# gue-ni/raytracer.glsl

Measured on AMD Instinct MI355X. Metric: Mpaths/s at 1920x1080, 8 bounces, 10k tris, higher is better.
Workload: dtype f32; 1 GPU; C2: 1920x1080, 8 bounces, 10000 triangles + 5 spheres, cube map 256^2, 1 spp/frame progressive, dof=1; parallelism=1 GPU(s), 8-row strips interleaved, gather to rank 0 every frame, frame_batch=1, kernel=4, wf_rays=4, wf_mode=1, wf_chunk=256, wf_early=0, wf_packed=0, mf_sets=4, mf_group_quads=32, mf_chunk_quads=32

## Files before the change

raytracer.glsl_amd/csrc/rt_mfma.hpp:

```cpp
#pragma once
#include "rt_wavefront.hpp"

#pragma clang fp contract(off)

namespace rt {

typedef __bf16 bf16x8 __attribute__((ext_vector_type(8)));
typedef float f32x16 __attribute__((ext_vector_type(16)));

constexpr int kMfTileTris = 10;
constexpr int kMfQuadTiles = 4;
constexpr int kMfQuadTris = kMfTileTris * kMfQuadTiles;
constexpr uint32_t kMfMaxChunkQuads = 32;
constexpr uint32_t kMfMaxGroupQuads = 64;

struct alignas(16) MfGroup {
    float cx, cy, cz;
    float E;
    float Ml;
    float Pw;
    float P;
    float pad1;
};

// ... 107 lines not shown

__device__ __forceinline__ float mf_margin(const MfGroup &G, float ncv, float no, const MfRay &r)
{
    float local = __builtin_fmaf(0.00396728515625f * G.E, ncv, 6.103515625e-05f * (G.Ml * r.wd));
    float cancel = 9.5367431640625e-07f * (__builtin_fmaf(G.E, no, G.P) * r.wd);
    float world = 9.5367431640625e-07f * __builtin_fmaf(G.E, r.wod, G.Pw * r.wd);
    return (local + cancel) + (world + 1e-30f);
}

struct alignas(16) MfCull {
    float cx, cy, cz, R;
    float ax, ay, az, Rc;
    float t1x, t1y, t1z, X;
    float t2x, t2y, t2z, Y;
    float Nmin, shape, hmin, lmax;
    float Pw, inv_len;
    float iB, iB2;
    float iB_lo, iB2_lo, pad0, pad1;
};
static_assert(sizeof(MfCull) == 112, "seven uint4 per tile");

__device__ __forceinline__ float wave_sum(float x) { for (int off = 32; off > 0; off >>= 1) x += __shfl_xor(x, off); return x; }

__global__ void __launch_bounds__(64) prepare_cull_kernel(const float4 *__restrict__ vertices, const uint32_t *__restrict__ visit_tri,
                                                          const uint32_t *__restrict__ order, uint32_t n_visits, uint32_t n_tiles, MfCull *__restrict__ out)
{
    const uint32_t q = blockIdx.x, lane = threadIdx.x;
    if (q >= n_tiles) return;
    const uint32_t pos = q * kMfTileTris + lane;
    const bool have = lane < (uint32_t)kMfTileTris && pos < n_visits;
    const float inf = __builtin_inff();
    f3 w[3] = {mk(0.0f, 0.0f, 0.0f), mk(0.0f, 0.0f, 0.0f), mk(0.0f, 0.0f, 0.0f)};
    if (have) { const uint32_t tri = visit_tri[order[pos]]; for (int k = 0; k < 3; ++k) { const float4 p = vertices[3 * (size_t)tri + k]; w[k] = mk(p.x, p.y, p.z); } }
    f3 lo = mk(inf, inf, inf), hi = mk(-inf, -inf, -inf);
    bool bad = false;
    if (have) for (int k = 0; k < 3; ++k) {
        lo = mk(fminf(lo.x, w[k].x), fminf(lo.y, w[k].y), fminf(lo.z, w[k].z));
        hi = mk(fmaxf(hi.x, w[k].x), fmaxf(hi.y, w[k].y), fmaxf(hi.z, w[k].z));
        bad |= !(fabsf(w[k].x) < 1e18f) || !(fabsf(w[k].y) < 1e18f) || !(fabsf(w[k].z) < 1e18f);
    }
    lo = mk(wave_min(lo.x), wave_min(lo.y), wave_min(lo.z));
    hi = mk(wave_max(hi.x), wave_max(hi.y), wave_max(hi.z));
    const f3 c = mk(0.5f * lo.x + 0.5f * hi.x, 0.5f * lo.y + 0.5f * hi.y, 0.5f * lo.z + 0.5f * hi.z);
    float R = 0.0f, Rc = 0.0f, E = 0.0f, Pw = 0.0f, Nmin = inf, shape = inf, hmin = inf;
    f3 nh = mk(0.0f, 0.0f, 0.0f);
    if (have) {
        const f3 e0 = w[1] - w[0], e1 = w[2] - w[1], e2 = w[0] - w[2];
        const f3 N = cross3(e0, mk(-e2.x, -e2.y, -e2.z));
        const float nn = __builtin_sqrtf(dot3(N, N));
        const float l0 = __builtin_sqrtf(dot3(e0, e0)), l1 = __builtin_sqrtf(dot3(e1, e1)), l2 = __builtin_sqrtf(dot3(e2, e2));
        for (int k = 0; k < 3; ++k) { const f3 r = w[k] - c; R = fmaxf(R, __builtin_sqrtf(dot3(r, r))); }
        { const f3 g = mk((w[0].x + w[1].x + w[2].x) * (1.0f / 3.0f), (w[0].y + w[1].y + w[2].y) * (1.0f / 3.0f), (w[0].z + w[1].z + w[2].z) * (1.0f / 3.0f)) - c;
          Rc = __builtin_sqrtf(dot3(g, g)); }
        E = fmaxf(l0, fmaxf(l1, l2));
        const float a0 = __builtin_sqrtf(dot3(w[0], w[0])), a1 = __builtin_sqrtf(dot3(w[1], w[1])), a2 = __builtin_sqrtf(dot3(w[2], w[2]));
        Pw = fmaxf(a0 * a1, fmaxf(a1 * a2, a2 * a0));
        Nmin = nn;
        nh = (nn > 0.0f) ? mk(N.x / nn, N.y / nn, N.z / nn) : mk(0.0f, 0.0f, 0.0f);
        const float c0 = -dot3(e0, e2) / (l0 * l2), c1 = -dot3(e1, e0) / (l1 * l0), c2 = -dot3(e2, e1) / (l2 * l1);
        const float cmax = fminf(1.0f, fmaxf(c0, fmaxf(c1, c2)));
        const float s = __builtin_sqrtf(fmaxf(0.0f, 0.5f * (1.0f - cmax)));
        const float lmin = fminf(l0, fminf(l1, l2));
        shape = (nn > 0.0f) ? 0.999f * s * lmin / nn : 0.0f;
        if (!(shape == shape)) shape = 0.0f;
        hmin = (E > 0.0f) ? 0.999f * nn / E : 0.0f;
        if (!(hmin == hmin)) hmin = 0.0f;
    }
    R = wave_max(R); Rc = wave_max(Rc); E = wave_max(E); Pw = wave_max(Pw); Nmin = wave_min(Nmin); shape = wave_min(shape); hmin = wave_min(hmin);
    bad = __any(bad) || __any(have && !(nh.x == nh.x && nh.y == nh.y && nh.z == nh.z));
    f3 a = mk(wave_sum(have ? nh.x : 0.0f), wave_sum(have ? nh.y : 0.0f), wave_sum(have ? nh.z : 0.0f));
    const float al = __builtin_sqrtf(dot3(a, a));
    a = (al > 0.0f) ? mk(a.x / al, a.y / al, a.z / al) : mk(0.0f, 0.0f, 1.0f);
    const float ca = have ? dot3(nh, a) : 1.0f;
    bad |= !(al > 0.0f) || __any(have && !(ca > 0.1f));
    const f3 ref = (fabsf(a.x) < 0.7f) ? mk(1.0f, 0.0f, 0.0f) : mk(0.0f, 1.0f, 0.0f);
    f3 b1 = cross3(a, ref);
    { const float bl = __builtin_sqrtf(dot3(b1, b1)); b1 = mk(b1.x / bl, b1.y / bl, b1.z / bl); }
    const f3 b2 = cross3(a, b1);
    const float ica = 1.0f / fmaxf(ca, 0.1f);
    const float gu = have ? dot3(nh, b1) * ica : 0.0f, gv = have ? dot3(nh, b2) * ica : 0.0f;
    const float suu = wave_sum(gu * gu), suv = wave_sum(gu * gv), svv = wave_sum(gv * gv);
    const float phi = 0.5f * atan2f(2.0f * suv, suu - svv);
    const float cp = cosf(phi), sp = sinf(phi);
    f3 t1 = mk(cp * b1.x + sp * b2.x, cp * b1.y + sp * b2.y, cp * b1.z + sp * b2.z);
    { const float tl = __builtin_sqrtf(dot3(t1, t1)); t1 = mk(t1.x / tl, t1.y / tl, t1.z / tl); }
    f3 t2 = cross3(a, t1);
    { const float tl = __builtin_sqrtf(dot3(t2, t2)); t2 = mk(t2.x / tl, t2.y / tl, t2.z / tl); }
    const float X = wave_max(have ? fabsf(dot3(nh, t1) * ica) : 0.0f), Y = wave_max(have ? fabsf(dot3(nh, t2) * ica) : 0.0f);
    if (lane != 0) return;
    MfCull rec;
    rec.cx = c.x; rec.cy = c.y; rec.cz = c.z; rec.R = R * 1.0001f + 1e-30f;
    rec.ax = a.x; rec.ay = a.y; rec.az = a.z; rec.Rc = Rc * 1.0001f + 1e-30f;
    rec.t1x = t1.x; rec.t1y = t1.y; rec.t1z = t1.z; rec.X = X * 1.001f + 1e-5f;
    rec.t2x = t2.x; rec.t2y = t2.y; rec.t2z = t2.z; rec.Y = Y * 1.001f + 1e-5f;
    bad |= !(rec.X < 16.0f) || !(rec.Y < 16.0f);
    rec.Nmin = bad ? 0.0f : Nmin * 0.999f; rec.shape = bad ? 0.0f : shape; rec.hmin = bad ? 0.0f : hmin; rec.lmax = E * 1.001f;
    rec.Pw = Pw * 1.001f;
    rec.inv_len = 0.9999f / __builtin_sqrtf(1.0f + rec.X * rec.X + rec.Y * rec.Y);
    rec.iB = 1.0001f / (1.0f + rec.X * rec.X); rec.iB2 = 1.0001f / (1.0f + rec.Y * rec.Y);
    rec.iB_lo = 0.9999f / (1.0f + rec.X * rec.X); rec.iB2_lo = 0.9999f / (1.0f + rec.Y * rec.Y);
    rec.pad0 = rec.pad1 = 0.0f;
    out[q] = rec;
}

struct MfPacket { f3 O, D; float ro, sigma, On; };

__device__ __forceinline__ float mf_max_dot(const MfCull &c, float wa, float w1, float w2, float wn)
{
    const bool inside = (wa > 0.0f) && (w1 <= c.X * wa) && (w2 <= c.Y * wa);
    const float num = __builtin_fmaf(c.Y, w2, __builtin_fmaf(c.X, w1, wa));
    const float corner = num * c.inv_len * (num > 0.0f ? 1.0003f : 1.0f);
// ... 49 lines not shown
```

raytracer.glsl_amd/csrc/rt_scan.hpp:

```cpp
#pragma once
#include <type_traits>
#include "rt_mfma.hpp"

#pragma clang fp contract(off)

namespace rt {

typedef uint32_t u32x4 __attribute__((ext_vector_type(4)));
typedef float f32x6 __attribute__((ext_vector_type(6)));

template <bool kMax> __device__ __forceinline__ float half_reduce(float x)
{
    auto op = [](float a, float b) { return kMax ? __builtin_fmaxf(a, b) : __builtin_fminf(a, b); };
    auto dpp = [](float v, auto ctrl) { return __builtin_bit_cast(float, __builtin_amdgcn_update_dpp(0, __builtin_bit_cast(int, v), decltype(ctrl)::value, 0xf, 0xf, false)); };
    x = op(x, dpp(x, std::integral_constant<int, 0xB1>{}));
    x = op(x, dpp(x, std::integral_constant<int, 0x4E>{}));
    x = op(x, dpp(x, std::integral_constant<int, 0x141>{}));
    x = op(x, dpp(x, std::integral_constant<int, 0x140>{}));
    const float r0 = __builtin_bit_cast(float, __builtin_amdgcn_readlane(__builtin_bit_cast(int, x), 0));
    const float r1 = __builtin_bit_cast(float, __builtin_amdgcn_readlane(__builtin_bit_cast(int, x), 16));
    return op(r0, r1);
}
__device__ __forceinline__ float half_max(float x) { return half_reduce<true>(x); }
__device__ __forceinline__ float half_min(float x) { return half_reduce<false>(x); }
template <bool kMax> __device__ __forceinline__ float full_reduce(float x)
{
    auto op = [](float a, float b) { return kMax ? __builtin_fmaxf(a, b) : __builtin_fminf(a, b); };
    auto dpp = [](float v, auto ctrl) { return __builtin_bit_cast(float, __builtin_amdgcn_update_dpp(0, __builtin_bit_cast(int, v), decltype(ctrl)::value, 0xf, 0xf, false)); };
    x = op(x, dpp(x, std::integral_constant<int, 0xB1>{}));
    x = op(x, dpp(x, std::integral_constant<int, 0x4E>{}));
    x = op(x, dpp(x, std::integral_constant<int, 0x141>{}));
    x = op(x, dpp(x, std::integral_constant<int, 0x140>{}));
    auto rl = [&](int l) { return __builtin_bit_cast(float, __builtin_amdgcn_readlane(__builtin_bit_cast(int, x), l)); };
    return op(op(rl(0), rl(16)), op(rl(32), rl(48)));
}

__global__ void __launch_bounds__(256) packet_cull_kernel(WaveBuffers wb, const MfCull *__restrict__ cull, uint32_t n_tiles, uint32_t bounce, float ro_add, float sigma_add)
{
    const uint32_t n_rays = wb.counts[bounce];
    const RayQueue qin = (bounce & 1u) ? wb.q[1] : wb.q[0];
    const uint32_t lane = threadIdx.x & 63u, n_gran = (n_rays + 127u) / 128u;
    const float inf = __builtin_inff();
    for (uint32_t g = blockIdx.x * 4u + (threadIdx.x >> 6); g < n_gran; g += gridDim.x * 4u) {
        f3 o[2], dh[2]; bool valid[2]; bool usable = true;
        f3 olo = mk(inf, inf, inf), ohi = mk(-inf, -inf, -inf), dlo = olo, dhi = ohi;
#pragma unroll
        for (int k = 0; k < 2; ++k) {
            const uint32_t slot = g * 128u + (uint32_t)k * 64u + lane;
            valid[k] = slot < n_rays;
            o[k] = mk(0.0f, 0.0f, 0.0f); dh[k] = o[k];
            if (valid[k]) {
                const float4 a = qin.a[slot], b = qin.b[slot];
                o[k] = mk(a.x, a.y, a.z);
                const f3 d = mk(a.w, b.x, b.y);
                const float dd = dot3(d, d), il = __builtin_amdgcn_rsqf(dd), dl = dd * il;
                dh[k] = mk(d.x * il, d.y * il, d.z * il);
                usable &= (dl > 0.0f) && (dl < inf) && (fabsf(o[k].x) < 1e18f) && (fabsf(o[k].y) < 1e18f) && (fabsf(o[k].z) < 1e18f);
                olo = mk(fminf(olo.x, o[k].x), fminf(olo.y, o[k].y), fminf(olo.z, o[k].z)); ohi = mk(fmaxf(ohi.x, o[k].x), fmaxf(ohi.y, o[k].y), fmaxf(ohi.z, o[k].z));
                dlo = mk(fminf(dlo.x, dh[k].x), fminf(dlo.y, dh[k].y), fminf(dlo.z, dh[k].z)); dhi = mk(fmaxf(dhi.x, dh[k].x), fmaxf(dhi.y, dh[k].y), fmaxf(dhi.z, dh[k].z));
            }
        }
        olo = mk(full_reduce<false>(olo.x), full_reduce<false>(olo.y), full_reduce<false>(olo.z)); ohi = mk(full_reduce<true>(ohi.x), full_reduce<true>(ohi.y), full_reduce<true>(ohi.z));
        dlo = mk(full_reduce<false>(dlo.x), full_reduce<false>(dlo.y), full_reduce<false>(dlo.z)); dhi = mk(full_reduce<true>(dhi.x), full_reduce<true>(dhi.y), full_reduce<true>(dhi.z));
        MfPacket pk;
        pk.O = mk(0.5f * olo.x + 0.5f * ohi.x, 0.5f * olo.y + 0.5f * ohi.y, 0.5f * olo.z + 0.5f * ohi.z);
        f3 D = mk(0.5f * dlo.x + 0.5f * dhi.x, 0.5f * dlo.y + 0.5f * dhi.y, 0.5f * dlo.z + 0.5f * dhi.z);
        const float DD = dot3(D, D), iDl = __builtin_amdgcn_rsqf(DD), Dl = DD * iDl;
        pk.D = mk(D.x * iDl, D.y * iDl, D.z * iDl);
        float ro = 0.0f, sigma = 0.0f;
#pragma unroll
        for (int k = 0; k < 2; ++k)
            if (valid[k]) {
                const f3 eo = o[k] - pk.O, ed = dh[k] - pk.D;
                ro = fmaxf(ro, __builtin_amdgcn_sqrtf(dot3(eo, eo))); sigma = fmaxf(sigma, __builtin_amdgcn_sqrtf(dot3(ed, ed)));
            }
        pk.ro = full_reduce<true>(ro) * 1.0001f + 1e-30f + ro_add; pk.sigma = full_reduce<true>(sigma) * 1.0001f + 2e-6f + sigma_add;
        usable = !__any(!usable) && (Dl > 0.25f);
        pk.On = __builtin_amdgcn_sqrtf(dot3(pk.O, pk.O)) * 1.0001f + pk.ro;
        uint32_t *const row = wb.keep + (size_t)g * wb.keep_words;
        MfCull c_next = {};
        bool have_next = usable && lane < n_tiles;
        if (have_next) c_next = cull[lane];
        for (uint32_t t0 = 0; t0 < n_tiles; t0 += 64u) {
            const MfCull c = c_next;
            const bool have_this = have_next;
            have_next = usable && t0 + 64u + lane < n_tiles;
            if (have_next) c_next = cull[t0 + 64u + lane];
            bool skip = false, open = false;
            f3 W = mk(0.0f, 0.0f, 0.0f); float L = 0.0f, nz = 0.0f, Wn = 0.0f;
            if (have_this && c.Nmin > 0.0f) {
                const f3 gq = pk.O - mk(c.cx, c.cy, c.cz);
                L = __builtin_amdgcn_sqrtf(dot3(gq, gq)) * 1.0001f;
                nz = 9.5367431640625e-07f * __builtin_fmaf(c.lmax, pk.On, c.Pw) * 1.01f;
                W = cross3(pk.D, gq);
                Wn = __builtin_amdgcn_sqrtf(dot3(W, W));
                skip = mf_certified_ka(c, pk, gq, L, nz, Wn);
                open = !skip;
            }
            if (__any(open)) { if (open) skip = mf_certified_b(c, pk, W, L, nz, Wn); }
            const unsigned long long have = (n_tiles - t0 >= 64u) ? ~0ull : ((1ull << (n_tiles - t0)) - 1ull);
            const unsigned long long keep = ~(unsigned long long)__builtin_amdgcn_ballot_w64(skip) & have;
            if (lane == 0u) {
                store_through(row + (t0 >> 5), (uint32_t)keep);
                if ((t0 >> 5) + 1u < wb.keep_words) store_through(row + ((t0 >> 5) + 1u), (uint32_t)(keep >> 32));
            }
        }
    }
}

__device__ __forceinline__ void exact_and_merge_at(const MfView &mf, const RayQueue &qin, unsigned long long *best, uint32_t slot, uint32_t pos)
{
    const float4 a = qin.a[slot], b = qin.b[slot];
    const uint32_t v = mf.order[pos];
    TriRay tr; tr.o = mk(a.x, a.y, a.z); tr.d = mk(a.w, b.x, b.y); tr.cv = cross3(tr.d, tr.o); tr.ncv = tr.nd = 0.0f;
    const float t = tri_exact(mf.edges_s[pos], mf.planes_s[pos], tr);
    if (kEps < t && t < kInf) atomicMin(&best[slot], ((unsigned long long)__float_as_uint(t) << 32) | v);
}

constexpr int kSoloSets = 4;
struct SoloCfg {
    static constexpr uint32_t kStepMax = 2u * 64u;
    static constexpr uint32_t kDrain = 192u;
// ... 668 lines not shown
```

raytracer.glsl_amd/csrc/rtgl_amd.hip:

```cpp
#include <hip/hip_runtime.h>
#include <algorithm>
#include <cmath>
#include <cstdio>
#include <cstring>
#include <string>
#include <vector>
#include <map>
#include <mutex>
#include <thread>
#include <condition_variable>
#include <memory>

#include "../../include/rtgl_amd.h"
#include "rt_device.hpp"
#include "rt_wavefront.hpp"
#include "rt_mfma.hpp"
#include "rt_scan.hpp"

#pragma clang fp contract(off)

using namespace rt;


__global__ void __launch_bounds__(256) prepare_triangles_kernel(const float4 *__restrict__ vertices,
// ... 125 lines not shown
    hipEvent_t ev0 = nullptr, ev1 = nullptr;
    bool timed = false;
    std::vector<hipEvent_t> kev;
    uint32_t kev_used = 0;
    std::vector<uint32_t> kev_frame_start;
    std::string error;

    std::vector<uint8_t> h_meshes, h_nodes, h_vertices;
    uint32_t n_meshes = 0, n_nodes = 0, n_vec4 = 0;

    SphereRec *d_spheres = nullptr; uint32_t n_spheres = 0;
    MaterialRec *d_materials = nullptr; uint32_t n_materials = 0;
    float4 *d_vertices = nullptr;
    uint32_t *d_sphere_visits = nullptr; uint32_t n_sphere_visits = 0;
    TriEdges *d_edges = nullptr; TriPlane *d_planes = nullptr; uint32_t n_tri_visits = 0;
    TriEdges *d_edges_s = nullptr; TriPlane *d_planes_s = nullptr;
    uint8_t *d_env = nullptr; int env_w = 0, env_h = 0, env_c = 0, env_faces = 0;
    float4 *d_image_own = nullptr, *d_image = nullptr;
    uint4 *d_rng = nullptr;
    Counters *d_counters = nullptr;
    uchar4 *d_u8 = nullptr;

    float2 *d_group_bounds = nullptr;
    MfGroup *d_mf_groups = nullptr; MfCull *d_mf_cull = nullptr; uint4 *d_mf_A = nullptr; uint32_t *d_mf_order = nullptr; uint32_t n_mf_groups = 0, mf_group_quads = 32; uint32_t *d_dbg_log = nullptr;
    void *d_wave = nullptr; size_t wave_capacity = 0; bool wave_multi = false;
    uint32_t *d_counts = nullptr; uint32_t counts_capacity = 0;
    uint32_t *h_counts = nullptr;
    hipEvent_t counts_ev = nullptr; bool counts_pending = false, counts_valid = false;
    bool timing_this_frame = false; uint32_t timing_frame_counter = 0;
    int kernel_in_use = -1;
    int n_cus = 256;
    uint2 *d_items = nullptr; size_t items_capacity = 0;
    uint32_t *d_sched = nullptr; size_t sched_capacity = 0;
    uint32_t *d_keep = nullptr; size_t keep_capacity = 0;
    uint32_t *d_keep0 = nullptr; size_t keep0_capacity = 0; bool keep0_valid = false; FrameParams keep0_params{}; uint32_t keep0_n0 = 0, keep0_words = 0; uint64_t keep0_scene = 0;
    uint64_t scene_version = 0;
    void *d_plan = nullptr; size_t plan_capacity = 0;
    void *d_stage = nullptr; size_t stage_capacity = 0;
    uint32_t *d_sort_hist = nullptr; uint32_t sort_bits_alloc = 0;
    int sort_set = 0; uint32_t sort_set_bits = 0; bool sort_sets_clean = false;
    float mesh_lo[3] = {0.0f, 0.0f, 0.0f}, mesh_hi[3] = {0.0f, 0.0f, 0.0f}, mesh_ext = 0.0f;
    uint2 *d_cand = nullptr; uint32_t cand_regions = 0, cand_region_pairs = 0, cand_region_target = 0; bool cand_fixed = false;
    bool solo_attr_set = false;
    bool group_explicit = false;
    bool kernel_explicit = false;
    uint32_t counts_n0 = 0, counts_len = 0;
    std::vector<uint32_t> est_counts;
// ... 168 lines not shown
            double cyc = 0, ticks = 0;
            for (int b = 0; b < 64 && h[16 * b + 8]; ++b) {
                const unsigned long long *d = h + 16 * b;
                fprintf(stderr, "rtgl clock bounce %2d: %llu waves, %.0f shader cycles per wave over %.0f ticks of 10 ns: %.3f GHz\n", b, d[8], (double)d[0] / d[8], (double)d[14] / d[8], d[14] ? (double)d[0] / (double)d[14] * 0.1 : 0.0);
                cyc += (double)d[0]; ticks += (double)d[14];
            }
            if (ticks > 0) fprintf(stderr, "rtgl clock: in-kernel shader clock of scan_solo_kernel, wave-time weighted over all launches: %.3f GHz\n", cyc / ticks * 0.1);
        }
#endif
        std::vector<unsigned long long> pc(16 * 64 * 2 * 16);
        if (hipMemcpy(pc.data(), reinterpret_cast<unsigned long long *>(ctx->d_dbg_log) + 2048, pc.size() * 8, hipMemcpyDeviceToHost) == hipSuccess)
            for (int b = 0; b < 8; ++b) {
                double tot = 0, cnt = 0; int nch = 0;
                for (int c = 0; c < 64; ++c) { const unsigned long long *e = pc.data() + ((size_t)16 * b * 64 + c) * 2; if (e[1]) { tot += (double)e[0]; cnt += (double)e[1]; nch = c + 1; } }
                if (cnt == 0) continue;
                fprintf(stderr, "rtgl stamps bounce %2d: mean wave time per chunk / bounce mean:", b);
                for (int c = 0; c < nch; ++c) { const unsigned long long *e = pc.data() + ((size_t)16 * b * 64 + c) * 2; fprintf(stderr, " %.2f", e[1] ? ((double)e[0] / (double)e[1]) / (tot / cnt) : 0.0); }
                fprintf(stderr, "\n");
            }
    }
#endif
    void *ptrs[] = { ctx->d_spheres, ctx->d_materials, ctx->d_vertices, ctx->d_sphere_visits, ctx->d_edges, ctx->d_planes,
                     ctx->d_env, ctx->d_image_own, ctx->d_rng, ctx->d_counters, ctx->d_u8, ctx->d_group_bounds, ctx->d_wave, ctx->d_counts, ctx->d_mf_groups, ctx->d_mf_A, ctx->d_mf_order,
                     ctx->d_dbg_log, ctx->d_cand, ctx->d_keep0, ctx->d_plan, ctx->d_stage, ctx->d_sort_hist, ctx->d_mf_cull, ctx->d_keep, ctx->d_items, ctx->d_sched, ctx->d_edges_s, ctx->d_planes_s, ctx->d_batch_rad };
    for (void *p : ptrs) if (p) (void)hipFree(p);
    for (hipEvent_t e : ctx->kev) (void)hipEventDestroy(e);
    if (ctx->h_counts) (void)hipHostFree(ctx->h_counts);
    if (ctx->counts_ev) (void)hipEventDestroy(ctx->counts_ev);
    if (ctx->ev0) (void)hipEventDestroy(ctx->ev0);
    if (ctx->ev1) (void)hipEventDestroy(ctx->ev1);
    if (ctx->own_stream) release_device_stream(ctx->device, ctx->own_stream, ctx->own_stream_shared);
    delete ctx;
}

extern "C" const char *rtgl_last_error(const rtgl_context *ctx) { return ctx ? ctx->error.c_str() : g_create_error.c_str(); }

static int flush_pending(rtgl_context *ctx);
#define ENTER_NOFLUSH(ctx) do { if (!(ctx)) return RTGL_ERR_INVALID; HIPCHK(ctx, hipSetDevice((ctx)->device)); } while (0)
#define ENTER(ctx) do { ENTER_NOFLUSH(ctx); if (!(ctx)->pending.empty()) { const int rcf_ = flush_pending(ctx); if (rcf_) return rcf_; } } while (0)
#define FANOUT(ctx, call) do { if (!(ctx)->parts.empty()) { (ctx)->gathered = false; \
    for (rtgl_context *part : (ctx)->parts) { const int rc_ = (call); if (rc_) return fail(ctx, rc_, std::string("device ") + std::to_string(part->device) + ": " + part->error); } \
    return RTGL_OK; } } while (0)

extern "C" int rtgl_create_multi(rtgl_context **out, int width, int height, const int *devices, int n_devices, int strip_rows)
{
    if (!out) return fail(nullptr, RTGL_ERR_INVALID, "out is NULL");
    *out = nullptr;
// ... 237 lines not shown
    while (!todo.empty()) {
        const size_t lo = todo.back().first, hi = todo.back().second, m = hi - lo;
        todo.pop_back();
        if (m <= (size_t)kMfTileTris) continue;
        const size_t unit = m > group_tris ? group_tris : (m > (size_t)kMfQuadTris ? (size_t)kMfQuadTris : (size_t)kMfTileTris);
        const size_t nl = ((m / 2 + unit - 1) / unit) * unit;
        const int dims = m > group_tris ? 3 : 6;
        float bl[6], bh[6];
        for (int a = 0; a < dims; ++a) { bl[a] = 3.0e38f; bh[a] = -3.0e38f; }
        for (size_t i = lo; i < hi; ++i)
            for (int a = 0; a < dims; ++a) { const float c = pts[6 * (size_t)order[i] + a]; bl[a] = std::min(bl[a], c); bh[a] = std::max(bh[a], c); }
        int ax = 0;
        for (int a = 1; a < dims; ++a) if (bh[a] - bl[a] > bh[ax] - bl[ax]) ax = a;
        std::nth_element(order.begin() + lo, order.begin() + lo + nl, order.begin() + hi, [&](uint32_t p, uint32_t q) {
            const float cp = pts[6 * (size_t)p + ax], cq = pts[6 * (size_t)q + ax];
            return cp < cq || (cp == cq && p < q);
        });
        todo.emplace_back(lo, lo + nl);
        todo.emplace_back(lo + nl, hi);
    }
    return order;
}

static int rebuild_triangles(rtgl_context *ctx)
{
    std::vector<uint32_t> visit_tri;
    uint32_t n_tris = ctx->n_vec4 / 3;
    for (uint32_t m = 0; m < ctx->n_meshes; ++m) {
        uint32_t start, size;
        memcpy(&start, ctx->h_meshes.data() + (size_t)m * 16, 4);
        memcpy(&size, ctx->h_meshes.data() + (size_t)m * 16 + 4, 4);
        uint64_t end = std::min<uint64_t>((uint64_t)start + size, n_tris);
        for (uint64_t t = start; t < end; ++t) visit_tri.push_back((uint32_t)t);
    }
    if (ctx->d_edges) { HIPCHK(ctx, hipFree(ctx->d_edges)); ctx->d_edges = nullptr; }
    if (ctx->d_planes) { HIPCHK(ctx, hipFree(ctx->d_planes)); ctx->d_planes = nullptr; }
    ctx->n_tri_visits = (uint32_t)visit_tri.size();
    ctx->scene_version++;
    {
        float lo[3] = {3.0e38f, 3.0e38f, 3.0e38f}, hi[3] = {-3.0e38f, -3.0e38f, -3.0e38f};
        const float *vx = reinterpret_cast<const float *>(ctx->h_vertices.data());
        for (uint32_t t : visit_tri)
            for (int k = 0; k < 3; ++k)
                for (int a = 0; a < 3; ++a) { const float c = vx[(size_t)t * 12 + 4 * k + a]; if (c == c && c > -1.0e30f && c < 1.0e30f) { lo[a] = std::min(lo[a], c); hi[a] = std::max(hi[a], c); } }
        ctx->mesh_ext = 0.0f;
        for (int a = 0; a < 3; ++a) { ctx->mesh_lo[a] = lo[a] <= hi[a] ? lo[a] : 0.0f; ctx->mesh_hi[a] = lo[a] <= hi[a] ? hi[a] : 0.0f; if (lo[a] <= hi[a]) ctx->mesh_ext = std::max(ctx->mesh_ext, hi[a] - lo[a]); }
    }
    if (ctx->n_tri_visits) {
        uint32_t *d_visit = nullptr;
        HIPCHK(ctx, hipMalloc((void **)&d_visit, visit_tri.size() * 4));
        HIPCHK(ctx, hipMemcpyAsync(d_visit, visit_tri.data(), visit_tri.size() * 4, hipMemcpyHostToDevice, ctx->stream));
        HIPCHK(ctx, hipMalloc((void **)&ctx->d_edges, (size_t)ctx->n_tri_visits * sizeof(TriEdges)));
        HIPCHK(ctx, hipMalloc((void **)&ctx->d_planes, (size_t)ctx->n_tri_visits * sizeof(TriPlane)));
        dim3 grid((ctx->n_tri_visits + 255) / 256);
        hipLaunchKernelGGL(prepare_triangles_kernel, grid, dim3(256), 0, ctx->stream, ctx->d_vertices, d_visit, ctx->n_tri_visits, ctx->d_edges, ctx->d_planes);
        HIPCHK(ctx, hipGetLastError());
        if (ctx->d_group_bounds) { HIPCHK(ctx, hipFree(ctx->d_group_bounds)); ctx->d_group_bounds = nullptr; }
        uint32_t n_groups = (ctx->n_tri_visits + kBoundGroup - 1) / kBoundGroup;
        HIPCHK(ctx, hipMalloc((void **)&ctx->d_group_bounds, (size_t)n_groups * sizeof(float2)));
        hipLaunchKernelGGL(group_bounds_kernel, dim3(n_groups), dim3(64), 0, ctx->stream, ctx->d_edges, ctx->n_tri_visits, ctx->d_group_bounds);
        HIPCHK(ctx, hipGetLastError());
        if (ctx->d_mf_groups) { HIPCHK(ctx, hipFree(ctx->d_mf_groups)); ctx->d_mf_groups = nullptr; }
        if (ctx->d_mf_A) { HIPCHK(ctx, hipFree(ctx->d_mf_A)); ctx->d_mf_A = nullptr; }
        if (ctx->d_mf_order) { HIPCHK(ctx, hipFree(ctx->d_mf_order)); ctx->d_mf_order = nullptr; }
        if (ctx->d_mf_cull) { HIPCHK(ctx, hipFree(ctx->d_mf_cull)); ctx->d_mf_cull = nullptr; }
        if (ctx->d_edges_s) { HIPCHK(ctx, hipFree(ctx->d_edges_s)); ctx->d_edges_s = nullptr; }
        if (ctx->d_planes_s) { HIPCHK(ctx, hipFree(ctx->d_planes_s)); ctx->d_planes_s = nullptr; }
        ctx->mf_group_quads = ctx->group_explicit ? (uint32_t)ctx->opt_mf_group_quads : 32u;
        const uint32_t group_tris = ctx->mf_group_quads * kMfQuadTris;
        ctx->n_mf_groups = (ctx->n_tri_visits + group_tris - 1) / group_tris;
        const std::vector<uint32_t> order = kd_order(ctx, visit_tri, group_tris);
        HIPCHK(ctx, hipMalloc((void **)&ctx->d_mf_order, order.size() * 4));
        HIPCHK(ctx, hipMemcpyAsync(ctx->d_mf_order, order.data(), order.size() * 4, hipMemcpyHostToDevice, ctx->stream));
        HIPCHK(ctx, hipMalloc((void **)&ctx->d_edges_s, (size_t)ctx->n_tri_visits * sizeof(TriEdges)));
        HIPCHK(ctx, hipMalloc((void **)&ctx->d_planes_s, (size_t)ctx->n_tri_visits * sizeof(TriPlane)));
        hipLaunchKernelGGL(gather_storage_order_kernel, dim3((ctx->n_tri_visits + 255) / 256), dim3(256), 0, ctx->stream, ctx->d_edges, ctx->d_planes, ctx->d_mf_order,
                           ctx->n_tri_visits, ctx->d_edges_s, ctx->d_planes_s);
        HIPCHK(ctx, hipMalloc((void **)&ctx->d_mf_groups, (size_t)ctx->n_mf_groups * sizeof(MfGroup)));
        const size_t a_bytes = ((size_t)ctx->n_mf_groups * ctx->mf_group_quads + 1) * kMfQuadTiles * 64 * sizeof(uint4);
        if (a_bytes > 0xFFFF0000ull) return fail(ctx, RTGL_ERR_INVALID, "mesh too large for the 32-bit tile offsets of the matrix-core scan");
        HIPCHK(ctx, hipMalloc((void **)&ctx->d_mf_A, a_bytes));
        HIPCHK(ctx, hipMemsetAsync(ctx->d_mf_A, 0, a_bytes, ctx->stream));
        hipLaunchKernelGGL(prepare_mfma_kernel, dim3(ctx->n_mf_groups), dim3(64), 0, ctx->stream, ctx->d_vertices, d_visit,
                           ctx->d_mf_order, ctx->n_tri_visits, ctx->n_mf_groups, ctx->mf_group_quads, ctx->d_mf_groups, ctx->d_mf_A, getenv("RTGL_AMD_ROW_GAMMA") ? (float)atof(getenv("RTGL_AMD_ROW_GAMMA")) : 1.220703125e-4f);
        HIPCHK(ctx, hipGetLastError());
        const uint32_t n_tiles_all = ctx->n_mf_groups * ctx->mf_group_quads * (uint32_t)kMfQuadTiles, n_tiles_alloc = n_tiles_all + 128u;
        HIPCHK(ctx, hipMalloc((void **)&ctx->d_mf_cull, (size_t)n_tiles_alloc * sizeof(MfCull)));
        HIPCHK(ctx, hipMemsetAsync(ctx->d_mf_cull, 0, (size_t)n_tiles_alloc * sizeof(MfCull), ctx->stream));
        hipLaunchKernelGGL(prepare_cull_kernel, dim3(n_tiles_all), dim3(64), 0, ctx->stream, ctx->d_vertices, d_visit,
                           ctx->d_mf_order, ctx->n_tri_visits, n_tiles_all, ctx->d_mf_cull);
        HIPCHK(ctx, hipGetLastError());
        HIPCHK(ctx, hipStreamSynchronize(ctx->stream));
        HIPCHK(ctx, hipFree(d_visit));
    } else ctx->n_mf_groups = 0;
    ctx->tris_dirty = false;
    return RTGL_OK;
}

static void kev_mark(rtgl_context *ctx)
{
    if (!ctx->timing_this_frame) return;
    if (ctx->kev_used == ctx->kev.size()) { hipEvent_t e; if (hipEventCreate(&e) != hipSuccess) return; ctx->kev.push_back(e); }
    (void)hipEventRecord(ctx->kev[ctx->kev_used++], ctx->stream);
}

static uint32_t solo_chunks(const rtgl_context *ctx);
static uint32_t solo_regions(const rtgl_context *ctx) { return std::max<uint32_t>((uint32_t)ctx->n_cus, solo_chunks(ctx)) * 8u; }

static size_t counts_bytes(uint32_t capacity) { return (size_t)(capacity + 1u) * sizeof(uint32_t); }

static void set_bin_cells(rtgl_context *ctx)
{
    WaveBuffers &wb = ctx->wb;
    const uint32_t T = wb.sort_T;
// ... 228 lines not shown
                               reinterpret_cast<const void *>(&scan_solo_kernel<false, 2, 3>), reinterpret_cast<const void *>(&scan_solo_kernel<true, 2, 3>)}) {
            hipFuncAttributes fattr;
            HIPCHK(ctx, hipFuncGetAttributes(&fattr, fn));
            HIPCHK(ctx, hipFuncSetAttribute(fn, hipFuncAttributeMaxDynamicSharedMemorySize, (int)(160 * 1024 - fattr.sharedSizeBytes)));
        }
        ctx->solo_attr_set = true;
    }

    if (cull) {
        float ro_add = 0.0f, sigma_add = 0.0f;
        bool have_bits = false;
        if (bounce == 0 && cam && camera_keep_widening(*cam, &ro_add, &sigma_add) && !getenv("RTGL_AMD_NO_CAMERA_KEEP")) {
            const size_t need = ((size_t)n0 / 128 + 16) * ctx->wb.keep_words;
            if (ctx->keep0_capacity < need) {
                if (ctx->d_keep0) { HIPCHK(ctx, hipFree(ctx->d_keep0)); ctx->d_keep0 = nullptr; }
                HIPCHK(ctx, hipMalloc((void **)&ctx->d_keep0, need * sizeof(uint32_t)));
                ctx->keep0_capacity = need; ctx->keep0_valid = false;
            }
            have_bits = ctx->keep0_valid && ctx->keep0_n0 == n0 && ctx->keep0_words == ctx->wb.keep_words && ctx->keep0_scene == ctx->scene_version && same_camera(ctx->keep0_params, *cam);
            ctx->wb.keep = ctx->d_keep0;
            if (!have_bits) { ctx->keep0_valid = true; ctx->keep0_n0 = n0; ctx->keep0_words = ctx->wb.keep_words; ctx->keep0_scene = ctx->scene_version; ctx->keep0_params = *cam; }
        } else { ctx->wb.keep = ctx->d_keep; ro_add = sigma_add = 0.0f; }
        if (!have_bits)
        hipLaunchKernelGGL(packet_cull_kernel, dim3(std::max(1u, std::min((est_gran + 3u) / 4u, 8192u))), dim3(256), 0, ctx->stream, ctx->wb, ctx->d_mf_cull, real_quads * (uint32_t)kMfQuadTiles, bounce, ro_add, sigma_add);
        if (dist == 2) {
            const uint32_t stride = n0 / Cfg::kRaysPerWave + 1u;
            const size_t off_tot = (((size_t)chunks * stride * sizeof(uint32_t)) + 255) & ~(size_t)255, off_base = (off_tot + (size_t)chunks * sizeof(uint32_t) + 255) & ~(size_t)255;
            const size_t need = off_base + ((size_t)chunks + 1) * sizeof(unsigned long long);
            if (ctx->plan_capacity < need) {
                if (ctx->d_plan) { HIPCHK(ctx, hipFree(ctx->d_plan)); ctx->d_plan = nullptr; }
                HIPCHK(ctx, hipMalloc(&ctx->d_plan, need));
                ctx->plan_capacity = need;
            }
            ctx->wb.plan_prefix = reinterpret_cast<uint32_t *>(ctx->d_plan); ctx->wb.plan_stride = stride;
            ctx->wb.plan_total = reinterpret_cast<uint32_t *>(reinterpret_cast<uint8_t *>(ctx->d_plan) + off_tot);
            ctx->wb.plan_base = reinterpret_cast<unsigned long long *>(reinterpret_cast<uint8_t *>(ctx->d_plan) + off_base);
            if (ctx->opt_counters) hipLaunchKernelGGL(scan_plan_kernel<true>, dim3(chunks), dim3(256), 0, ctx->stream, ctx->wb, bounce, chunk_quads, real_quads, ctx->d_counters);
            else hipLaunchKernelGGL(scan_plan_kernel<false>, dim3(chunks), dim3(256), 0, ctx->stream, ctx->wb, bounce, chunk_quads, real_quads, ctx->d_counters);
            hipLaunchKernelGGL(scan_plan_base_kernel, dim3(1), dim3(64), 0, ctx->stream, ctx->wb, chunks);
        }
        if (dynamic) {
        const uint32_t stride = n0 / Cfg::kRaysPerWave + 1u;
        const size_t head = ((size_t)ctx->wb.sched_stride * sizeof(uint32_t) + 255) & ~(size_t)255, need = head + (size_t)chunks * stride * sizeof(uint32_t);
        if (ctx->items_capacity < need) {
            if (ctx->d_items) { HIPCHK(ctx, hipFree(ctx->d_items)); ctx->d_items = nullptr; }
            HIPCHK(ctx, hipMalloc((void **)&ctx->d_items, need));
            ctx->items_capacity = need;
// ... 572 lines not shown
```

Measured before the change: 826.4 Mpaths/s.

## Add two-level hierarchical culling with node records over groups of tiles

Builds coarser cull records (nodes covering 16 tiles by default) using a generalized prepare kernel that loops over many triangles per record. The packet cull kernel first tests each ray packet against node records, compacts the surviving nodes into LDS, then tests only the tiles inside open nodes and assembles the keep bitmask in shared memory. The aim is to avoid testing every tile's cull record for every packet when large regions can be rejected at once. In exchange it adds extra passes, LDS atomics and wave syncs, and the looser node bounds may reject less than the per-tile tests.

Measured after the change: 844.2 Mpaths/s (median of 6 runs). 2.2% higher.

```diff
diff --git a/raytracer.glsl_amd/csrc/rt_mfma.hpp b/raytracer.glsl_amd/csrc/rt_mfma.hpp
--- a/raytracer.glsl_amd/csrc/rt_mfma.hpp
+++ b/raytracer.glsl_amd/csrc/rt_mfma.hpp
@@ -153,71 +153,110 @@
 
 __device__ __forceinline__ float wave_sum(float x) { for (int off = 32; off > 0; off >>= 1) x += __shfl_xor(x, off); return x; }
 
+struct CullTri { f3 w[3]; };
+__device__ __forceinline__ CullTri cull_tri_at(const float4 *__restrict__ vertices, const uint32_t *__restrict__ visit_tri, const uint32_t *__restrict__ order, uint32_t pos)
+{
+    CullTri t;
+    const uint32_t tri = visit_tri[order[pos]];
+    for (int k = 0; k < 3; ++k) { const float4 p = vertices[3 * (size_t)tri + k]; t.w[k] = mk(p.x, p.y, p.z); }
+    return t;
+}
+__device__ __forceinline__ f3 cull_unit_normal(const CullTri &t, float *nn_out)
+{
+    const f3 e0 = t.w[1] - t.w[0], e2 = t.w[0] - t.w[2];
+    const f3 N = cross3(e0, mk(-e2.x, -e2.y, -e2.z));
+    const float nn = __builtin_sqrtf(dot3(N, N));
+    if (nn_out) *nn_out = nn;
+    return (nn > 0.0f) ? mk(N.x / nn, N.y / nn, N.z / nn) : mk(0.0f, 0.0f, 0.0f);
+}
+
 __global__ void __launch_bounds__(64) prepare_cull_kernel(const float4 *__restrict__ vertices, const uint32_t *__restrict__ visit_tri,
-                                                          const uint32_t *__restrict__ order, uint32_t n_visits, uint32_t n_tiles, MfCull *__restrict__ out)
+                                                          const uint32_t *__restrict__ order, uint32_t n_visits, uint32_t n_recs, uint32_t rec_tris,
+                                                          MfCull *__restrict__ out)
 {
     const uint32_t q = blockIdx.x, lane = threadIdx.x;
-    if (q >= n_tiles) return;
-    const uint32_t pos = q * kMfTileTris + lane;
-    const bool have = lane < (uint32_t)kMfTileTris && pos < n_visits;
+    if (q >= n_recs) return;
+    const uint64_t p_begin = (uint64_t)q * rec_tris, p_end = min(p_begin + rec_tris, (uint64_t)n_visits);
     const float inf = __builtin_inff();
-    f3 w[3] = {mk(0.0f, 0.0f, 0.0f), mk(0.0f, 0.0f, 0.0f), mk(0.0f, 0.0f, 0.0f)};
-    if (have) { const uint32_t tri = visit_tri[order[pos]]; for (int k = 0; k < 3; ++k) { const float4 p = vertices[3 * (size_t)tri + k]; w[k] = mk(p.x, p.y, p.z); } }
     f3 lo = mk(inf, inf, inf), hi = mk(-inf, -inf, -inf);
     bool bad = false;
-    if (have) for (int k = 0; k < 3; ++k) {
-        lo = mk(fminf(lo.x, w[k].x), fminf(lo.y, w[k].y), fminf(lo.z, w[k].z));
-        hi = mk(fmaxf(hi.x, w[k].x), fmaxf(hi.y, w[k].y), fmaxf(hi.z, w[k].z));
-        bad |= !(fabsf(w[k].x) < 1e18f) || !(fabsf(w[k].y) < 1e18f) || !(fabsf(w[k].z) < 1e18f);
+    for (uint64_t p = p_begin + lane; p < p_end; p += 64u) {
+        const CullTri t = cull_tri_at(vertices, visit_tri, order, (uint32_t)p);
+        for (int k = 0; k < 3; ++k) {
+            lo = mk(fminf(lo.x, t.w[k].x), fminf(lo.y, t.w[k].y), fminf(lo.z, t.w[k].z));
+            hi = mk(fmaxf(hi.x, t.w[k].x), fmaxf(hi.y, t.w[k].y), fmaxf(hi.z, t.w[k].z));
+            bad |= !(fabsf(t.w[k].x) < 1e18f) || !(fabsf(t.w[k].y) < 1e18f) || !(fabsf(t.w[k].z) < 1e18f);
+        }
     }
     lo = mk(wave_min(lo.x), wave_min(lo.y), wave_min(lo.z));
     hi = mk(wave_max(hi.x), wave_max(hi.y), wave_max(hi.z));
     const f3 c = mk(0.5f * lo.x + 0.5f * hi.x, 0.5f * lo.y + 0.5f * hi.y, 0.5f * lo.z + 0.5f * hi.z);
     float R = 0.0f, Rc = 0.0f, E = 0.0f, Pw = 0.0f, Nmin = inf, shape = inf, hmin = inf;
-    f3 nh = mk(0.0f, 0.0f, 0.0f);
-    if (have) {
+    f3 nsum = mk(0.0f, 0.0f, 0.0f);
+    bool nan_normal = false;
+    for (uint64_t p = p_begin + lane; p < p_end; p += 64u) {
+        const CullTri t = cull_tri_at(vertices, visit_tri, order, (uint32_t)p);
+        const f3 *w = t.w;
         const f3 e0 = w[1] - w[0], e1 = w[2] - w[1], e2 = w[0] - w[2];
-        const f3 N = cross3(e0, mk(-e2.x, -e2.y, -e2.z));
-        const float nn = __builtin_sqrtf(dot3(N, N));
+        float nn;
+        const f3 nh = cull_unit_normal(t, &nn);
         const float l0 = __builtin_sqrtf(dot3(e0, e0)), l1 = __builtin_sqrtf(dot3(e1, e1)), l2 = __builtin_sqrtf(dot3(e2, e2));
         for (int k = 0; k < 3; ++k) { const f3 r = w[k] - c; R = fmaxf(R, __builtin_sqrtf(dot3(r, r))); }
         { const f3 g = mk((w[0].x + w[1].x + w[2].x) * (1.0f / 3.0f), (w[0].y + w[1].y + w[2].y) * (1.0f / 3.0f), (w[0].z + w[1].z + w[2].z) * (1.0f / 3.0f)) - c;
-          Rc = __builtin_sqrtf(dot3(g, g)); }
-        E = fmaxf(l0, fmaxf(l1, l2));
+          Rc = fmaxf(Rc, __builtin_sqrtf(dot3(g, g))); }
+        const float El = fmaxf(l0, fmaxf(l1, l2));
+        E = fmaxf(E, El);
         const float a0 = __builtin_sqrtf(dot3(w[0], w[0])), a1 = __builtin_sqrtf(dot3(w[1], w[1])), a2 = __builtin_sqrtf(dot3(w[2], w[2]));
-        Pw = fmaxf(a0 * a1, fmaxf(a1 * a2, a2 * a0));
-        Nmin = nn;
-        nh = (nn > 0.0f) ? mk(N.x / nn, N.y / nn, N.z / nn) : mk(0.0f, 0.0f, 0.0f);
+        Pw = fmaxf(Pw, fmaxf(a0 * a1, fmaxf(a1 * a2, a2 * a0)));
+        Nmin = fminf(Nmin, nn);
+        nan_normal |= !(nh.x == nh.x && nh.y == nh.y && nh.z == nh.z);
         const float c0 = -dot3(e0, e2) / (l0 * l2), c1 = -dot3(e1, e0) / (l1 * l0), c2 = -dot3(e2, e1) / (l2 * l1);
         const float cmax = fminf(1.0f, fmaxf(c0, fmaxf(c1, c2)));
         const float s = __builtin_sqrtf(fmaxf(0.0f, 0.5f * (1.0f - cmax)));
         const float lmin = fminf(l0, fminf(l1, l2));
-        shape = (nn > 0.0f) ? 0.999f * s * lmin / nn : 0.0f;
-        if (!(shape == shape)) shape = 0.0f;
-        hmin = (E > 0.0f) ? 0.999f * nn / E : 0.0f;
-        if (!(hmin == hmin)) hmin = 0.0f;
+        float sh = (nn > 0.0f) ? 0.999f * s * lmin / nn : 0.0f;
+        if (!(sh == sh)) sh = 0.0f;
+        float hm = (El > 0.0f) ? 0.999f * nn / El : 0.0f;
+        if (!(hm == hm)) hm = 0.0f;
+        shape = fminf(shape, sh); hmin = fminf(hmin, hm);
+        nsum = mk(nsum.x + nh.x, nsum.y + nh.y, nsum.z + nh.z);
     }
     R = wave_max(R); Rc = wave_max(Rc); E = wave_max(E); Pw = wave_max(Pw); Nmin = wave_min(Nmin); shape = wave_min(shape); hmin = wave_min(hmin);
-    bad = __any(bad) || __any(have && !(nh.x == nh.x && nh.y == nh.y && nh.z == nh.z));
-    f3 a = mk(wave_sum(have ? nh.x : 0.0f), wave_sum(have ? nh.y : 0.0f), wave_sum(have ? nh.z : 0.0f));
+    bad = __any(bad) || __any(nan_normal);
+    f3 a = mk(wave_sum(nsum.x), wave_sum(nsum.y), wave_sum(nsum.z));
     const float al = __builtin_sqrtf(dot3(a, a));
     a = (al > 0.0f) ? mk(a.x / al, a.y / al, a.z / al) : mk(0.0f, 0.0f, 1.0f);
-    const float ca = have ? dot3(nh, a) : 1.0f;
-    bad |= !(al > 0.0f) || __any(have && !(ca > 0.1f));
     const f3 ref = (fabsf(a.x) < 0.7f) ? mk(1.0f, 0.0f, 0.0f) : mk(0.0f, 1.0f, 0.0f);
     f3 b1 = cross3(a, ref);
     { const float bl = __builtin_sqrtf(dot3(b1, b1)); b1 = mk(b1.x / bl, b1.y / bl, b1.z / bl); }
     const f3 b2 = cross3(a, b1);
-    const float ica = 1.0f / fmaxf(ca, 0.1f);
-    const float gu = have ? dot3(nh, b1) * ica : 0.0f, gv = have ? dot3(nh, b2) * ica : 0.0f;
-    const float suu = wave_sum(gu * gu), suv = wave_sum(gu * gv), svv = wave_sum(gv * gv);
+    bool spread = false;
+    float suu = 0.0f, suv = 0.0f, svv = 0.0f;
+    for (uint64_t p = p_begin + lane; p < p_end; p += 64u) {
+        const CullTri t = cull_tri_at(vertices, visit_tri, order, (uint32_t)p);
+        const f3 nh = cull_unit_normal(t, nullptr);
+        const float ca = dot3(nh, a);
+        spread |= !(ca > 0.1f);
+        const float ica = 1.0f / fmaxf(ca, 0.1f);
+        const float gu = dot3(nh, b1) * ica, gv = dot3(nh, b2) * ica;
+        suu += gu * gu; suv += gu * gv; svv += gv * gv;
+    }
+    bad |= !(al > 0.0f) || __any(spread);
+    suu = wave_sum(suu); suv = wave_sum(suv); svv = wave_sum(svv);
     const float phi = 0.5f * atan2f(2.0f * suv, suu - svv);
     const float cp = cosf(phi), sp = sinf(phi);
     f3 t1 = mk(cp * b1.x + sp * b2.x, cp * b1.y + sp * b2.y, cp * b1.z + sp * b2.z);
     { const float tl = __builtin_sqrtf(dot3(t1, t1)); t1 = mk(t1.x / tl, t1.y / tl, t1.z / tl); }
     f3 t2 = cross3(a, t1);
     { const float tl = __builtin_sqrtf(dot3(t2, t2)); t2 = mk(t2.x / tl, t2.y / tl, t2.z / tl); }
-    const float X = wave_max(have ? fabsf(dot3(nh, t1) * ica) : 0.0f), Y = wave_max(have ? fabsf(dot3(nh, t2) * ica) : 0.0f);
+    float X = 0.0f, Y = 0.0f;
+    for (uint64_t p = p_begin + lane; p < p_end; p += 64u) {
+        const CullTri t = cull_tri_at(vertices, visit_tri, order, (uint32_t)p);
+        const f3 nh = cull_unit_normal(t, nullptr);
+        const float ica = 1.0f / fmaxf(dot3(nh, a), 0.1f);
+        X = fmaxf(X, fabsf(dot3(nh, t1) * ica)); Y = fmaxf(Y, fabsf(dot3(nh, t2) * ica));
+    }
+    X = wave_max(X); Y = wave_max(Y);
     if (lane != 0) return;
     MfCull rec;
     rec.cx = c.x; rec.cy = c.y; rec.cz = c.z; rec.R = R * 1.0001f + 1e-30f;
diff --git a/raytracer.glsl_amd/csrc/rt_scan.hpp b/raytracer.glsl_amd/csrc/rt_scan.hpp
--- a/raytracer.glsl_amd/csrc/rt_scan.hpp
+++ b/raytracer.glsl_amd/csrc/rt_scan.hpp
@@ -35,8 +35,30 @@
     return op(op(rl(0), rl(16)), op(rl(32), rl(48)));
 }
 
-__global__ void __launch_bounds__(256) packet_cull_kernel(WaveBuffers wb, const MfCull *__restrict__ cull, uint32_t n_tiles, uint32_t bounce, float ro_add, float sigma_add)
-{
+constexpr uint32_t kCullRowWords = 128;
+__device__ __forceinline__ void wave_lds_sync() { __builtin_amdgcn_fence(__ATOMIC_ACQ_REL, "wavefront"); __builtin_amdgcn_wave_barrier(); }
+__device__ __forceinline__ bool cull_lane(const MfCull &c, bool have, const MfPacket &pk)
+{
+    bool skip = false, open = false;
+    f3 W = mk(0.0f, 0.0f, 0.0f); float L = 0.0f, nz = 0.0f, Wn = 0.0f;
+    if (have && c.Nmin > 0.0f) {
+        const f3 gq = pk.O - mk(c.cx, c.cy, c.cz);
+        L = __builtin_amdgcn_sqrtf(dot3(gq, gq)) * 1.0001f;
+        nz = 9.5367431640625e-07f * __builtin_fmaf(c.lmax, pk.On, c.Pw) * 1.01f;
+        W = cross3(pk.D, gq);
+        Wn = __builtin_amdgcn_sqrtf(dot3(W, W));
+        skip = mf_certified_ka(c, pk, gq, L, nz, Wn);
+        open = !skip;
+    }
+    if (__any(open)) { if (open) skip = mf_certified_b(c, pk, W, L, nz, Wn); }
+    return skip;
+}
+
+__global__ void __launch_bounds__(256) packet_cull_kernel(WaveBuffers wb, const MfCull *__restrict__ cull, uint32_t n_tiles, uint32_t bounce, float ro_add, float sigma_add,
+                                                          const MfCull *__restrict__ node, uint32_t node_shift)
+{
+    __shared__ uint32_t s_row[4][kCullRowWords];
+    __shared__ uint32_t s_open[4][64];
     const uint32_t n_rays = wb.counts[bounce];
     const RayQueue qin = (bounce & 1u) ? wb.q[1] : wb.q[0];
     const uint32_t lane = threadIdx.x & 63u, n_gran = (n_rays + 127u) / 128u;
@@ -78,6 +100,45 @@
         usable = !__any(!usable) && (Dl > 0.25f);
         pk.On = __builtin_amdgcn_sqrtf(dot3(pk.O, pk.O)) * 1.0001f + pk.ro;
         uint32_t *const row = wb.keep + (size_t)g * wb.keep_words;
+        if (node_shift) {
+            const uint32_t wv = threadIdx.x >> 6, S = 1u << node_shift, n_nodes = (n_tiles + S - 1u) >> node_shift;
+            const uint32_t batch_nodes = (kCullRowWords * 32u) >> node_shift;
+            const uint32_t grp = min(S, 32u);
+            for (uint32_t b0 = 0; b0 < n_nodes; b0 += batch_nodes) {
+                const uint32_t tile0 = b0 << node_shift, w0 = tile0 >> 5;
+                s_row[wv][lane] = 0u; s_row[wv][lane + 64u] = 0u;
+                wave_lds_sync();
+                for (uint32_t n0 = b0; n0 < min(b0 + batch_nodes, n_nodes); n0 += 64u) {
+                    const bool have_node = usable && n0 + lane < n_nodes;
+                    MfCull c = {};
+                    if (have_node) c = node[n0 + lane];
+                    const bool closed = cull_lane(c, have_node, pk);
+                    const unsigned long long open_nodes = __builtin_amdgcn_ballot_w64(n0 + lane < n_nodes && !closed);
+                    if (n0 + lane < n_nodes && !closed)
+                        s_open[wv][__builtin_amdgcn_mbcnt_hi((uint32_t)(open_nodes >> 32), __builtin_amdgcn_mbcnt_lo((uint32_t)open_nodes, 0u))] = n0 + lane;
+                    wave_lds_sync();
+                    const uint32_t n_items = (uint32_t)__builtin_popcountll(open_nodes) << node_shift;
+                    for (uint32_t i0 = 0; i0 < n_items; i0 += 64u) {
+                        const uint32_t j = i0 + lane;
+                        const uint32_t t = j < n_items ? (s_open[wv][j >> node_shift] << node_shift) + (j & (S - 1u)) : n_tiles;
+                        const bool have_tile = t < n_tiles;
+                        MfCull ct = {};
+                        if (usable && have_tile) ct = cull[t];
+                        const bool skip = cull_lane(ct, usable && have_tile, pk);
+                        const unsigned long long keep = __builtin_amdgcn_ballot_w64(have_tile && !skip);
+                        if (j < n_items && (lane & (grp - 1u)) == 0u) {
+                            const uint32_t bits = (uint32_t)(keep >> lane) & (uint32_t)((1ull << grp) - 1ull);
+                            if (bits) atomicOr(&s_row[wv][(t >> 5) - w0], bits << (t & 31u));
+                        }
+                    }
+                    wave_lds_sync();
+                }
+                for (uint32_t k = lane; k < kCullRowWords && w0 + k < wb.keep_words; k += 64u)
+                    store_through(row + w0 + k, s_row[wv][k]);
+                wave_lds_sync();
+            }
+            continue;
+        }
         MfCull c_next = {};
         bool have_next = usable && lane < n_tiles;
         if (have_next) c_next = cull[lane];
@@ -86,18 +147,7 @@
             const bool have_this = have_next;
             have_next = usable && t0 + 64u + lane < n_tiles;
             if (have_next) c_next = cull[t0 + 64u + lane];
-            bool skip = false, open = false;
-            f3 W = mk(0.0f, 0.0f, 0.0f); float L = 0.0f, nz = 0.0f, Wn = 0.0f;
-            if (have_this && c.Nmin > 0.0f) {
-                const f3 gq = pk.O - mk(c.cx, c.cy, c.cz);
-                L = __builtin_amdgcn_sqrtf(dot3(gq, gq)) * 1.0001f;
-                nz = 9.5367431640625e-07f * __builtin_fmaf(c.lmax, pk.On, c.Pw) * 1.01f;
-                W = cross3(pk.D, gq);
-                Wn = __builtin_amdgcn_sqrtf(dot3(W, W));
-                skip = mf_certified_ka(c, pk, gq, L, nz, Wn);
-                open = !skip;
-            }
-            if (__any(open)) { if (open) skip = mf_certified_b(c, pk, W, L, nz, Wn); }
+            const bool skip = cull_lane(c, have_this, pk);
             const unsigned long long have = (n_tiles - t0 >= 64u) ? ~0ull : ((1ull << (n_tiles - t0)) - 1ull);
             const unsigned long long keep = ~(unsigned long long)__builtin_amdgcn_ballot_w64(skip) & have;
             if (lane == 0u) {
diff --git a/raytracer.glsl_amd/csrc/rtgl_amd.hip b/raytracer.glsl_amd/csrc/rtgl_amd.hip
--- a/raytracer.glsl_amd/csrc/rtgl_amd.hip
+++ b/raytracer.glsl_amd/csrc/rtgl_amd.hip
@@ -171,7 +171,7 @@
     uchar4 *d_u8 = nullptr;
 
     float2 *d_group_bounds = nullptr;
-    MfGroup *d_mf_groups = nullptr; MfCull *d_mf_cull = nullptr; uint4 *d_mf_A = nullptr; uint32_t *d_mf_order = nullptr; uint32_t n_mf_groups = 0, mf_group_quads = 32; uint32_t *d_dbg_log = nullptr;
+    MfGroup *d_mf_groups = nullptr; MfCull *d_mf_cull = nullptr; MfCull *d_mf_cull_node = nullptr; uint32_t cull_node_shift = 0; uint4 *d_mf_A = nullptr; uint32_t *d_mf_order = nullptr; uint32_t n_mf_groups = 0, mf_group_quads = 32; uint32_t *d_dbg_log = nullptr;
     void *d_wave = nullptr; size_t wave_capacity = 0; bool wave_multi = false;
     uint32_t *d_counts = nullptr; uint32_t counts_capacity = 0;
     uint32_t *h_counts = nullptr;
@@ -386,7 +386,7 @@
 #endif
     void *ptrs[] = { ctx->d_spheres, ctx->d_materials, ctx->d_vertices, ctx->d_sphere_visits, ctx->d_edges, ctx->d_planes,
                      ctx->d_env, ctx->d_image_own, ctx->d_rng, ctx->d_counters, ctx->d_u8, ctx->d_group_bounds, ctx->d_wave, ctx->d_counts, ctx->d_mf_groups, ctx->d_mf_A, ctx->d_mf_order,
-                     ctx->d_dbg_log, ctx->d_cand, ctx->d_keep0, ctx->d_plan, ctx->d_stage, ctx->d_sort_hist, ctx->d_mf_cull, ctx->d_keep, ctx->d_items, ctx->d_sched, ctx->d_edges_s, ctx->d_planes_s, ctx->d_batch_rad };
+                     ctx->d_dbg_log, ctx->d_cand, ctx->d_keep0, ctx->d_plan, ctx->d_stage, ctx->d_sort_hist, ctx->d_mf_cull, ctx->d_mf_cull_node, ctx->d_keep, ctx->d_items, ctx->d_sched, ctx->d_edges_s, ctx->d_planes_s, ctx->d_batch_rad };
     for (void *p : ptrs) if (p) (void)hipFree(p);
     for (hipEvent_t e : ctx->kev) (void)hipEventDestroy(e);
     if (ctx->h_counts) (void)hipHostFree(ctx->h_counts);
@@ -670,6 +670,13 @@
     return order;
 }
 
+static uint32_t cull_node_shift_option()
+{
+    uint32_t shift = 4;
+    if (const char *e = getenv("RTGL_AMD_CULL_NODE")) { const long v = atol(e); shift = v <= 0 ? 0u : v <= 8 ? 2u : v <= 32 ? 4u : 6u; }
+    return shift;
+}
+
 static int rebuild_triangles(rtgl_context *ctx)
 {
     std::vector<uint32_t> visit_tri;
@@ -712,6 +719,7 @@
         if (ctx->d_mf_A) { HIPCHK(ctx, hipFree(ctx->d_mf_A)); ctx->d_mf_A = nullptr; }
         if (ctx->d_mf_order) { HIPCHK(ctx, hipFree(ctx->d_mf_order)); ctx->d_mf_order = nullptr; }
         if (ctx->d_mf_cull) { HIPCHK(ctx, hipFree(ctx->d_mf_cull)); ctx->d_mf_cull = nullptr; }
+        if (ctx->d_mf_cull_node) { HIPCHK(ctx, hipFree(ctx->d_mf_cull_node)); ctx->d_mf_cull_node = nullptr; }
         if (ctx->d_edges_s) { HIPCHK(ctx, hipFree(ctx->d_edges_s)); ctx->d_edges_s = nullptr; }
         if (ctx->d_planes_s) { HIPCHK(ctx, hipFree(ctx->d_planes_s)); ctx->d_planes_s = nullptr; }
         ctx->mf_group_quads = ctx->group_explicit ? (uint32_t)ctx->opt_mf_group_quads : 32u;
@@ -736,8 +744,16 @@
         HIPCHK(ctx, hipMalloc((void **)&ctx->d_mf_cull, (size_t)n_tiles_alloc * sizeof(MfCull)));
         HIPCHK(ctx, hipMemsetAsync(ctx->d_mf_cull, 0, (size_t)n_tiles_alloc * sizeof(MfCull), ctx->stream));
         hipLaunchKernelGGL(prepare_cull_kernel, dim3(n_tiles_all), dim3(64), 0, ctx->stream, ctx->d_vertices, d_visit,
-                           ctx->d_mf_order, ctx->n_tri_visits, n_tiles_all, ctx->d_mf_cull);
+                           ctx->d_mf_order, ctx->n_tri_visits, n_tiles_all, (uint32_t)kMfTileTris, ctx->d_mf_cull);
         HIPCHK(ctx, hipGetLastError());
+        ctx->cull_node_shift = cull_node_shift_option();
+        if (ctx->cull_node_shift) {
+            const uint32_t n_nodes_all = (n_tiles_all + (1u << ctx->cull_node_shift) - 1u) >> ctx->cull_node_shift;
+            HIPCHK(ctx, hipMalloc((void **)&ctx->d_mf_cull_node, (size_t)n_nodes_all * sizeof(MfCull)));
+            hipLaunchKernelGGL(prepare_cull_kernel, dim3(n_nodes_all), dim3(64), 0, ctx->stream, ctx->d_vertices, d_visit,
+                               ctx->d_mf_order, ctx->n_tri_visits, n_nodes_all, (uint32_t)kMfTileTris << ctx->cull_node_shift, ctx->d_mf_cull_node);
+            HIPCHK(ctx, hipGetLastError());
+        }
         HIPCHK(ctx, hipStreamSynchronize(ctx->stream));
         HIPCHK(ctx, hipFree(d_visit));
     } else ctx->n_mf_groups = 0;
@@ -1012,7 +1028,8 @@
             if (!have_bits) { ctx->keep0_valid = true; ctx->keep0_n0 = n0; ctx->keep0_words = ctx->wb.keep_words; ctx->keep0_scene = ctx->scene_version; ctx->keep0_params = *cam; }
         } else { ctx->wb.keep = ctx->d_keep; ro_add = sigma_add = 0.0f; }
         if (!have_bits)
-        hipLaunchKernelGGL(packet_cull_kernel, dim3(std::max(1u, std::min((est_gran + 3u) / 4u, 8192u))), dim3(256), 0, ctx->stream, ctx->wb, ctx->d_mf_cull, real_quads * (uint32_t)kMfQuadTiles, bounce, ro_add, sigma_add);
+        hipLaunchKernelGGL(packet_cull_kernel, dim3(std::max(1u, std::min((est_gran + 3u) / 4u, 8192u))), dim3(256), 0, ctx->stream, ctx->wb, ctx->d_mf_cull, real_quads * (uint32_t)kMfQuadTiles, bounce, ro_add, sigma_add,
+                           ctx->d_mf_cull_node, ctx->d_mf_cull_node ? ctx->cull_node_shift : 0u);
         if (dist == 2) {
             const uint32_t stride = n0 / Cfg::kRaysPerWave + 1u;
             const size_t off_tot = (((size_t)chunks * stride * sizeof(uint32_t)) + 255) & ~(size_t)255, off_base = (off_tot + (size_t)chunks * sizeof(uint32_t) + 255) & ~(size_t)255;
```
